# dingliumath/MCMC.jl

Hardware: AMD Instinct MI355X
Metric: MCMC steps*chains/sec (1M chains, d=32) (higher is better)
Workload: dtype f64; 1 GPU; metric: d=32 iso-Normal, RWM(0.1), 2^20 chains/GPU (BASELINE metric); SerialMC(steps=2967, burnin=296, thinning=10), 1048576 chains/GPU, RWM; d=32, chains_per_gpu=1048576, global_chains=1048576, sampler=rwm, burnin=296, thinning=10, kept_per_chain=268, steps_per_launch=0, evals=3111124992, key=metric|d=32|chains=1048576|rwm|steps=2967|thinning=10|spl=0, parallelism=chains sharded over 1 GPU(s), no collective in the step loop

## Files before the change

### mcmc.jl_amd/csrc/detmath.hpp

```cpp
#pragma once
#include <hip/hip_runtime.h>
#include <stdint.h>

#include "bm_log_table.inc"
#include "erfc_table.inc"
#include "softplus_table.inc"

namespace mcmc {

enum : uint32_t { TAG_NORMAL = 0u, TAG_ACCEPT = 1u, TAG_NUTS_DOUBLING = 3u, TAG_NUTS_MERGE = 4u, TAG_DATA = 7u };

struct u32x4 { uint32_t x, y, z, w; };

template <bool U = false>
__device__ __forceinline__ u32x4 philox4x32_10(uint32_t c0, uint32_t c1, uint32_t c2, uint32_t c3,
                                               uint32_t k0, uint32_t k1) {
#pragma unroll
    for (int r = 0; r < 10; ++r) {
        if (r > 0) { k0 += 0x9E3779B9u; k1 += 0xBB67AE85u; }
        const uint64_t p0 = (uint64_t)0xD2511F53u * (uint64_t)c0;
        const uint64_t p1 = (uint64_t)0xCD9E8D57u * (uint64_t)c2;
        uint32_t n0, n2;
        if (U && r == 0) {
            n0 = (uint32_t)(p1 >> 32) ^ (c1 ^ k0);
// ... 99 lines not shown
    const double ln2_hi = 0x1.62e42fee00000p-1;
    const double ln2_lo = 0x1.a39ef35793c76p-33;
    const double shifter = 0x1.8p52;
    const double xc = __builtin_fmin(__builtin_fmax(x, -746.0), 710.0);
    const double t = __builtin_fma(xc, inv_ln2, shifter);
    const double kd = t - shifter;
    E.k = (int)kd;
    double r = __builtin_fma(-kd, ln2_hi, xc);
    E.r = __builtin_fma(-kd, ln2_lo, r);
    E.x = x;
    E.p = 0x1.6124613a86d09p-33;
}
__device__ __forceinline__ void det_exp_s2(ExpState& E) {
    double p = E.p;
    const double r = E.r;
    p = __builtin_fma(p, r, 0x1.1eed8eff8d898p-29);
    p = __builtin_fma(p, r, 0x1.ae64567f544e4p-26);
    p = __builtin_fma(p, r, 0x1.27e4fb7789f5cp-22);
    p = __builtin_fma(p, r, 0x1.71de3a556c734p-19);
    p = __builtin_fma(p, r, 0x1.a01a01a01a01ap-16);
    p = __builtin_fma(p, r, 0x1.a01a01a01a01ap-13);
    p = __builtin_fma(p, r, 0x1.6c16c16c16c17p-10);
    E.p = p;
}
__device__ __forceinline__ void det_exp_s3(ExpState& E) {
    double p = E.p;
    const double r = E.r;
    p = __builtin_fma(p, r, 0x1.1111111111111p-7);
    p = __builtin_fma(p, r, 0x1.5555555555555p-5);
    p = __builtin_fma(p, r, 0x1.5555555555555p-3);
    p = __builtin_fma(p, r, 0.5);
    p = __builtin_fma(p, r, 1.0);
    p = __builtin_fma(p, r, 1.0);
    E.p = p;
}
__device__ __forceinline__ double det_exp_fin(const ExpState& E) {
    const int k1 = E.k / 2, k2 = E.k - k1;
    double res = (E.p * pow2i(k1)) * pow2i(k2);
    const double x = E.x;
    if (x > 709.782712893384) res = __builtin_inf();
    if (x < -745.1332191019412) res = 0.0;
    if (x != x) res = x;
    return res;
}
__device__ __forceinline__ double det_exp(double x) {
    ExpState E;
    det_exp_s1(x, E);
    det_exp_s2(E);
    det_exp_s3(E);
    return det_exp_fin(E);
}

__device__ __forceinline__ void det_sincos2pi(double u, double& s_out, double& c_out) {
    const double q = __builtin_floor(__builtin_fma(u, 4.0, 0.5));
    const double r = __builtin_fma(q, -0.25, u);
    const double r2 = r * r;
    double S = -0x1.6fadb9f155744p-1;
    S = __builtin_fma(S, r2, 0x1.e8f434d018d63p+1);
    S = __builtin_fma(S, r2, -0x1.e3074fde8871fp+3);
    S = __builtin_fma(S, r2, 0x1.50783487ee782p+5);
    S = __builtin_fma(S, r2, -0x1.32d2cce62bd86p+6);
    S = __builtin_fma(S, r2, 0x1.466bc6775aae2p+6);
    S = __builtin_fma(S, r2, -0x1.4abbce625be53p+5);
    S = __builtin_fma(S, r2, 0x1.921fb54442d18p+2);
    double C = 0x1.20c62c2f2d7f5p-2;
    C = __builtin_fma(C, r2, -0x1.b6e24f44b128fp+0);
    C = __builtin_fma(C, r2, 0x1.f9d38a3763cc3p+2);
    C = __builtin_fma(C, r2, -0x1.a6d1f2a204a8cp+4);
    C = __builtin_fma(C, r2, 0x1.e1f506891babbp+5);
    C = __builtin_fma(C, r2, -0x1.55d3c7e3cbffap+6);
    C = __builtin_fma(C, r2, 0x1.03c1f081b5ac4p+6);
    C = __builtin_fma(C, r2, -0x1.3bd3cc9be45dep+4);
    C = __builtin_fma(C, r2, 1.0);
    const double sn = r * S;
    const int qi = ((int)q) & 3;
    const double a = (qi & 1) ? C : sn;
    const double b = (qi & 1) ? sn : C;
    s_out = (qi & 2) ? -a : a;
    c_out = (qi == 1 || qi == 2) ? -b : b;
}

static __device__ const double kBmLogTab[128][4] = {BM_LOG_TABLE_ROWS};
static __device__ const double kBmLog512Tab[512][4] = {BM_LOG512_TABLE_ROWS};

__device__ __forceinline__ double bm_log_u32(uint32_t w, const double (*tab)[4] = kBmLog512Tab) {
    const double ln2_hi = 0x1.62e42fee00000p-1;
    const double ln2_lo = 0x1.a39ef35793c76p-33;
    const double x = (double)w + 0.5;
    const uint64_t b = d2bits(x);
    const uint32_t xh = (uint32_t)(b >> 32);
    const uint32_t up = (xh >> 19) & 1u;
    const int e = (int)(xh >> 20) + (int)up - (1023 + 32);
    const uint32_t mhi = ((0x3ffu ^ up) << 20) | (xh & 0x000fffffu);
    const double m = bits2d(((uint64_t)mhi << 32) | (b & 0xffffffffull));
    typedef double f64x2_t __attribute__((ext_vector_type(2)));
    const f64x2_t* row = reinterpret_cast<const f64x2_t*>(reinterpret_cast<const char*>(tab) + ((xh >> 6) & 0x3fe0u));
    const f64x2_t a = row[0], t = row[1];
    const double r = __builtin_fma(m, a.x, -1.0);
    double P = __builtin_fma(r, -0x1.5555555555555p-3, 0x1.999999999999ap-3);
    P = __builtin_fma(r, P, -0x1p-2);
    P = __builtin_fma(r, P, 0x1.5555555555555p-2);
    P = __builtin_fma(r, P, -0x1p-1);
    const double p = __builtin_fma(r * r, P, r);
    const double de = (double)e;
    const double hi = __builtin_fma(de, ln2_hi, a.y);
    const double lo = __builtin_fma(de, ln2_lo, t.x) + p;
    return hi + lo;
}

static __device__ const double kBmRad512Tab[512][4] = {BM_RAD512_TABLE_ROWS};

__device__ __forceinline__ double bm_rad2_u32(uint32_t w, const double (*tab)[4] = kBmRad512Tab) {
    const double m2ln2_hi = -0x1.62e42fee00000p+0;
    const double m2ln2_lo = -0x1.a39ef35793c76p-32;
    const double x = (double)w + 0.5;
    const uint64_t b = d2bits(x);
    const uint32_t xh = (uint32_t)(b >> 32);
    const uint32_t up = (xh >> 19) & 1u;
    const int e = (int)(xh >> 20) + (int)up - (1023 + 32);
    const uint32_t mhi = ((0x3ffu ^ up) << 20) | (xh & 0x000fffffu);
    const double m = bits2d(((uint64_t)mhi << 32) | (b & 0xffffffffull));
    typedef double f64x2_t __attribute__((ext_vector_type(2)));
    const f64x2_t* row = reinterpret_cast<const f64x2_t*>(reinterpret_cast<const char*>(tab) + ((xh >> 6) & 0x3fe0u));
    const f64x2_t a = row[0], t = row[1];
    const double r2 = __builtin_fma(m, a.x, 2.0);
    double Q = __builtin_fma(r2, 0x1.5555555555555p-8, 0x1.999999999999ap-7);
    Q = __builtin_fma(r2, Q, 0x1p-5);
    Q = __builtin_fma(r2, Q, 0x1.5555555555555p-4);
    Q = __builtin_fma(r2, Q, 0x1p-2);
    const double p2 = __builtin_fma(r2 * r2, Q, r2);
    const double de = (double)e;
    const double hi = __builtin_fma(de, m2ln2_hi, a.y);
    const double lo = __builtin_fma(de, m2ln2_lo, t.x) + p2;
    return hi + lo;
}

static __device__ const double kBmRadPTab[4 * BM_RADP_NROWS][2] = {BM_RADP_TABLE_ROWS};
static __device__ const double kBmRadTTab[4 * BM_RADT_NROWS][2] = {BM_RADT_TABLE_ROWS};

struct RadTab {
    const double (*d)[2];
    bool lds;
};
__device__ __forceinline__ RadTab rad_tab_global() { return RadTab{kBmRadPTab, false}; }

__device__ __forceinline__ double bm_radius_u32(uint32_t w, RadTab rt) {
    typedef double f64x2_t __attribute__((ext_vector_type(2)));
    const uint32_t sm = (uint32_t)((int32_t)w >> 31);
    const uint32_t v = w ^ sm;
    const double y = (double)v;
    const uint64_t b = d2bits(y);
    const uint32_t yh = (uint32_t)(b >> 32);
    const bool tail = v < (1u << 21);
    constexpr uint32_t kOff0 = 0u - ((uint32_t)((1023 + 21) << 5) << 4);
    constexpr uint32_t kOff1 = kOff0 + (uint32_t)(BM_RADP_NROWS / 2) * 16u;
    uint32_t sel;
    asm("v_bfi_b32 %0, %1, %2, %3" : "=v"(sel) : "v"(sm), "v"(kOff1), "s"(kOff0));
    uint32_t off;
    asm("v_lshl_add_u32 %0, %1, 4, %2" : "=v"(off) : "v"(yh >> 15), "v"(sel));
    uint32_t th = yh;
    asm("v_and_or_b32 %0, %0, %1, %2" : "+v"(th) : "s"(0x7fffu), "v"(0x3ff00000u));
    if (!rt.lds) off = tail ? 0u : off;
    double t = bits2d(((uint64_t)th << 32) | (b & 0xffffffffull)) - (1.0 + 1.0 / 64.0);
    const char* base = reinterpret_cast<const char*>(rt.d) + off;
    f64x2_t c0 = *reinterpret_cast<const f64x2_t*>(base);
    f64x2_t c1 = *reinterpret_cast<const f64x2_t*>(base + 16 * BM_RADP_NROWS);
    f64x2_t c2 = *reinterpret_cast<const f64x2_t*>(base + 32 * BM_RADP_NROWS);
    f64x2_t c3 = *reinterpret_cast<const f64x2_t*>(base + 48 * BM_RADP_NROWS);
    if (tail) {
        uint32_t vv = v;
        asm volatile("" : "+v"(vv));
        const double x = (double)vv + 0.5;
        const uint64_t bx = d2bits(x);
        const uint32_t xh = (uint32_t)(bx >> 32);
        const uint32_t rw = (uint32_t)((int)(xh >> 15) - ((1023 - 1) << 5)) * 16u + (sm & (16u * (BM_RADT_NROWS / 2)));
        t = bits2d(((uint64_t)((xh & 0x7fffu) | 0x3ff00000u) << 32) | (bx & 0xffffffffull)) - (1.0 + 1.0 / 64.0);
        asm volatile(
            "global_load_dwordx4 %0, %4, %5\n\t"
            "global_load_dwordx4 %1, %4, %6\n\t"
            "global_load_dwordx4 %2, %4, %7\n\t"
            "global_load_dwordx4 %3, %4, %8\n\t"
            "s_waitcnt vmcnt(0)"
            : "=&v"(c0), "=&v"(c1), "=&v"(c2), "=&v"(c3)
            : "v"(rw), "s"(&kBmRadTTab[0][0]), "s"(&kBmRadTTab[BM_RADT_NROWS][0]),
              "s"(&kBmRadTTab[2 * BM_RADT_NROWS][0]), "s"(&kBmRadTTab[3 * BM_RADT_NROWS][0])
            : "memory");
    }
    double q = __builtin_fma(c3.y, t, c3.x);
    q = __builtin_fma(q, t, c2.y);
    q = __builtin_fma(q, t, c2.x);
    q = __builtin_fma(q, t, c1.y);
    q = __builtin_fma(q, t, c1.x);
    q = __builtin_fma(q, t, c0.y);
    double r = __builtin_fma(q, t, c0.x);
    asm volatile("" : "+v"(r));
    return r;
}

typedef double dm_f64x2 __attribute__((ext_vector_type(2)));

static __device__ const double kExp2Tab[64][2] = {EXP2_TABLE_ROWS};

struct ExpTState {
    double x, r, em;
    dm_f64x2 t;
    int e;
};
__device__ __forceinline__ void det_exp_tab_s1(double x, ExpTState& E, const double (*tab)[2] = kExp2Tab) {
    const double k64 = 0x1.71547652b82fep+6;
    const double l_hi = 0x1.62e42fee00000p-7;
    const double l_lo = 0x1.a39ef35793c76p-39;
    const double shifter = 0x1.8p52;
    const double xc = __builtin_fmin(__builtin_fmax(x, -746.0), 710.0);
    const double kd = __builtin_fma(xc, k64, shifter) - shifter;
    const int k = (int)kd;
    E.t = *reinterpret_cast<const dm_f64x2*>(tab[k & 63]);
    E.e = k >> 6;
    const double r = __builtin_fma(-kd, l_hi, xc);
    E.r = __builtin_fma(-kd, l_lo, r);
    E.x = x;
}
__device__ __forceinline__ void det_exp_tab_s2(ExpTState& E) {
    const double r = E.r;
    double P = __builtin_fma(r, 0x1.6c16c16c16c17p-10, 0x1.1111111111111p-7);
    P = __builtin_fma(r, P, 0x1.5555555555555p-5);
    P = __builtin_fma(r, P, 0x1.5555555555555p-3);
    P = __builtin_fma(r, P, 0.5);
    P = __builtin_fma(r, P, 1.0);
    E.em = r * P;
}
__device__ __forceinline__ double det_exp_tab_fin(const ExpTState& E) {
    const int e1 = E.e / 2, e2 = E.e - e1;
    double res = E.t.x + __builtin_fma(E.t.x, E.em, E.t.y);
    res = (res * pow2i(e1)) * pow2i(e2);
    return E.x != E.x ? E.x : res;
}
__device__ __forceinline__ double det_exp_tab(double x, const double (*tab)[2] = kExp2Tab) {
    ExpTState E;
    det_exp_tab_s1(x, E, tab);
    det_exp_tab_s2(E);
    return det_exp_tab_fin(E);
}

struct LogTState {
    double v, m, p;
    dm_f64x2 a, t;
    int e;
};
#ifndef GLM_LOG_FREXP
#define GLM_LOG_FREXP 0
#endif
__device__ __forceinline__ void det_log_tab_s1(double v, LogTState& L, const double (*tab)[4] = kBmLogTab) {
#if GLM_LOG_FREXP
    const double mh = __builtin_amdgcn_frexp_mant(v);
    const int eh = __builtin_amdgcn_frexp_exp(v);
    const uint64_t b = d2bits(mh);
    const uint32_t top7 = (uint32_t)(b >> 45) & 0x7fu;
    const uint32_t up = top7 >> 6;
    L.e = eh - 1 + (int)up;
    L.m = bits2d((b & 0x000fffffffffffffull) | ((uint64_t)(0x3ffu - up) << 52));
    const dm_f64x2* row = reinterpret_cast<const dm_f64x2*>(tab[top7]);
    L.a = row[0];
    L.t = row[1];
    L.v = v;
#else
    const bool sub = v < 0x1p-1022;
    const double xs = sub ? v * 0x1p54 : v;
    const uint64_t b = d2bits(xs);
    const uint32_t top7 = (uint32_t)(b >> 45) & 0x7fu;
    const uint32_t up = top7 >> 6;
    L.e = (int)(uint32_t)(b >> 52) - 1023 + (int)up - (sub ? 54 : 0);
    L.m = bits2d((b & 0x000fffffffffffffull) | ((uint64_t)(0x3ffu - up) << 52));
    const dm_f64x2* row = reinterpret_cast<const dm_f64x2*>(tab[top7]);
    L.a = row[0];
    L.t = row[1];
    L.v = v;
#endif
}
__device__ __forceinline__ void det_log_tab_s2(LogTState& L) {
    const double r = __builtin_fma(L.m, L.a.x, -1.0);
    double P = __builtin_fma(r, -0x1p-3, 0x1.2492492492492p-3);
    P = __builtin_fma(r, P, -0x1.5555555555555p-3);
    P = __builtin_fma(r, P, 0x1.999999999999ap-3);
    P = __builtin_fma(r, P, -0x1p-2);
    P = __builtin_fma(r, P, 0x1.5555555555555p-2);
    P = __builtin_fma(r, P, -0x1p-1);
    L.p = __builtin_fma(r * r, P, r);
}
__device__ __forceinline__ double det_log_tab_fin(const LogTState& L) {
    const double ln2_hi = 0x1.62e42fee00000p-1;
    const double ln2_lo = 0x1.a39ef35793c76p-33;
    const double de = (double)L.e;
    const double hi = __builtin_fma(de, ln2_hi, L.a.y);
    const double lo = __builtin_fma(de, ln2_lo, L.t.x) + L.p;
    const double res = L.v == 0.0 ? -__builtin_inf() : hi + lo;
    return L.v != L.v ? L.v : res;
}
__device__ __forceinline__ double det_log_tab(double v, const double (*tab)[4] = kBmLogTab) {
    LogTState L;
    det_log_tab_s1(v, L, tab);
    det_log_tab_s2(L);
    return det_log_tab_fin(L);
}

static __device__ const double kSoftplusTab[SP_NROWS][10] = {SP_TABLE_ROWS};


struct LogiState {
    double u, t, p, d;
    const dm_f64x2* row;
};
__device__ __forceinline__ void det_logi_s1(double eta, double w, LogiState& S, const double (*tab)[10] = kSoftplusTab) {
    const double shifter = 0x1.8p52;
    const double u = -(w * eta);
    const double vs = __builtin_fmin(__builtin_fabs(u), (double)SP_VMAX);
    const double tt = __builtin_fma(vs, (double)SP_SEG, shifter);
    const uint32_t j = (uint32_t)d2bits(tt);
    const double kd = tt - shifter;
    S.t = __builtin_fma(-kd, 1.0 / SP_SEG, vs);
    S.row = reinterpret_cast<const dm_f64x2*>(tab[j]);
    S.u = u;
}
__device__ __forceinline__ void det_logi_s2(LogiState& S) {
    const double t = S.t;
    const dm_f64x2 c89 = S.row[4], c67 = S.row[3], c45 = S.row[2];
    double p = c89.y, d = c89.y;
    p = __builtin_fma(p, t, c89.x);
    d = __builtin_fma(d, t, p); p = __builtin_fma(p, t, c67.y);
    d = __builtin_fma(d, t, p); p = __builtin_fma(p, t, c67.x);
    d = __builtin_fma(d, t, p); p = __builtin_fma(p, t, c45.y);
    d = __builtin_fma(d, t, p); p = __builtin_fma(p, t, c45.x);
    S.p = p;
    S.d = d;
}
__device__ __forceinline__ void det_logi_fin(const LogiState& S, double w, double& term, double& rv) {
    const double t = S.t;
    const dm_f64x2 c23 = S.row[1], c01 = S.row[0];
    double p = S.p, d = S.d;
    d = __builtin_fma(d, t, p); p = __builtin_fma(p, t, c23.y);
    d = __builtin_fma(d, t, p); p = __builtin_fma(p, t, c23.x);
    d = __builtin_fma(d, t, p); p = __builtin_fma(p, t, c01.y);
    d = __builtin_fma(d, t, p); p = __builtin_fma(p, t, c01.x);
    term = -(__builtin_fmax(S.u, 0.0) + p);
    const double sig = S.u >= 0.0 ? 1.0 + d : -d;
    rv = w * sig;
}
__device__ __forceinline__ void det_logi(double eta, double w, double& term, double& rv,
                                         const double (*tab)[10] = kSoftplusTab) {
    LogiState S;
    det_logi_s1(eta, w, S, tab);
    det_logi_s2(S);
    det_logi_fin(S, w, term, rv);
}

static __device__ const double kBmSinCos1024Tab[1024][2] = {BM_SINCOS1024_TABLE_ROWS};

constexpr double kSinJ1 = 0x1.921fb54442d18p-30, kSinJ3 = -0x1.4abbce625be53p-91, kSinJ5 = 0x1.466bc6775aae2p-154;
constexpr double kCosJ2 = -0x1.3bd3cc9be45dep-60, kCosJ4 = 0x1.03c1f081b5ac4p-122;

__device__ __forceinline__ void det_sincos2pi_u32(uint32_t w, double& s_out, double& c_out,
                                                  const double (*sct)[2] = kBmSinCos1024Tab) {
    const int32_t ji = ((int32_t)(w << 10)) >> 10;
    const uint32_t off = (w - (uint32_t)ji) >> 18;
    const double j = (double)ji;
    const double j2 = j * j;
    const double sr = j * __builtin_fma(j2, __builtin_fma(j2, kSinJ5, kSinJ3), kSinJ1);
    const double cr = __builtin_fma(j2, __builtin_fma(j2, kCosJ4, kCosJ2), 1.0);
    typedef double f64x2_t __attribute__((ext_vector_type(2)));
    const f64x2_t a = *reinterpret_cast<const f64x2_t*>(reinterpret_cast<const char*>(sct) + off);
    s_out = __builtin_fma(a.x, cr, a.y * sr);
    c_out = __builtin_fma(a.y, cr, -(a.x * sr));
}

__device__ __forceinline__ double sqrt_pos_normal(double x) {
    const double y = __builtin_amdgcn_rsq(x);
    double g = x * y;
    double h = 0.5 * y;
    const double r = __builtin_fma(-h, g, 0.5);
    g = __builtin_fma(g, r, g);
    h = __builtin_fma(h, r, h);
    double e = __builtin_fma(-g, g, x);
    g = __builtin_fma(e, h, g);
    e = __builtin_fma(-g, g, x);
    return __builtin_fma(e, h, g);
}

__device__ __forceinline__ void normals4(const u32x4& w, double& z0, double& z1, double& z2, double& z3,
                                         RadTab rt = rad_tab_global(),
                                         const double (*sct)[2] = kBmSinCos1024Tab) {
    {
        const double rad = bm_radius_u32(w.x, rt);
        double s, c;
        det_sincos2pi_u32(w.y, s, c, sct);
        z0 = rad * c; z1 = rad * s;
    }
    {
        const double rad = bm_radius_u32(w.z, rt);
        double s, c;
        det_sincos2pi_u32(w.w, s, c, sct);
        z2 = rad * c; z3 = rad * s;
    }
    asm volatile("" : "+v"(z0), "+v"(z1), "+v"(z2), "+v"(z3));
}

__device__ __attribute__((noinline)) bool gt_det_log_exact(double ratio, double u) { return ratio > det_log(u); }
__device__ __forceinline__ bool gt_det_log(double ratio, double u) {
    const double L = (double)__builtin_amdgcn_logf((float)u) * 0x1.62e42fefa39efp-1;
    const double E = 0x1p-16 * (1.0 + __builtin_fabs(L));
    const bool sure_acc = ratio > L + E;
    const bool sure_rej = ratio <= L - E;
    bool acc = sure_acc;
    if (!sure_acc && !sure_rej) acc = gt_det_log_exact(ratio, u);
    return acc;
}

__device__ __forceinline__ double round_away(double x) {
    double t = __builtin_trunc(x);
    const double fr = x - t;
    if (fr >= 0.5) t += 1.0;
    else if (fr <= -0.5) t -= 1.0;
    return t;
}

static __device__ const double kErfcTaylor[14] = {ERFC_TAYLOR_COEFS};
static __device__ const double kErfcPoly[32][13] = {ERFC_POLY_ROWS};
__device__ __forceinline__ double det_erfcx_ge_half(double x) {
    if (x >= 128.0) {
        const double v = 1.0 / (x * x);
        const double s = __builtin_fma(__builtin_fma(__builtin_fma(v, -1.875, 0.75), v, -0.5), v, 1.0);
        return s / (x * 0x1.c5bf891b4ef6bp+0);
    }
    const uint64_t bx = d2bits(x);
    const uint32_t hx = (uint32_t)(bx >> 32);
    const int i = (int)(hx >> 18) - (1022 << 2);
    const double c = bits2d((uint64_t)((hx & 0xfffc0000u) | 0x00020000u) << 32);
    const double sc = bits2d((uint64_t)(2046u - (hx >> 20) + 3u) << 52);
    const double t = (x - c) * sc;
    const double* P = kErfcPoly[i];
    double p = P[12];
#pragma unroll
    for (int n = 11; n >= 0; --n) p = __builtin_fma(p, t, P[n]);
    return p;
}
__device__ __forceinline__ double det_erfc(double a) {
    const double x = __builtin_fabs(a);
    double r;
    if (x < 0.5) {
        const double u = x * x;
        double q = kErfcTaylor[13];
#pragma unroll
        for (int n = 12; n >= 0; --n) q = __builtin_fma(q, u, kErfcTaylor[n]);
        r = 1.0 - x * q;
    } else if (x < 32.0) {
        const double p = det_erfcx_ge_half(x);
        const double xh = bits2d(d2bits(x) & 0xfffffffff8000000ull);
        const double e1 = det_exp(-(xh * xh));
        const double e2 = det_exp(-((x - xh) * (x + xh)));
        r = (e1 * e2) * p;
    } else {
        r = 0.0;
    }
    r = a < 0.0 ? 2.0 - r : r;
    return a != a ? a : r;
}
__device__ __forceinline__ double det_log1p(double t) {
    const double u = 1.0 + t;
    return u == 1.0 ? t : det_log(u) * (t / (u - 1.0));
}
__device__ __forceinline__ double det_normlogcdf(double z) {
    const double invsqrt2 = 0x1.6a09e667f3bcdp-1;
    const double r = z < -1.0 ? det_log(det_erfcx_ge_half(-z * invsqrt2) / 2.0) - (z * z) / 2.0
                              : det_log1p(-det_erfc(z * invsqrt2) / 2.0);
    return z != z ? z : r;
}

}
```

### mcmc.jl_amd/csrc/samplers.hpp

```cpp
#pragma once
#include "common.hpp"
#include "detmath.hpp"
#include "models.hpp"
#include "ram.hpp"
#include "host/kernels_api.hpp"

namespace mcmc {

constexpr int kBlock = 256;

enum TabMode : int { kTabLds = 0, kTabGlobal = 1 };

struct BmLds {
    double (*rd)[2];
    double (*sc)[2];
};
__device__ __forceinline__ BmLds bm_lds_tables() {
    __shared__ __attribute__((aligned(16))) double lds_radd[4 * BM_RADP_NROWS][2];
    __shared__ __attribute__((aligned(16))) double lds_sct[1024][2];
    return BmLds{lds_radd, lds_sct};
}

template <int NT>
__device__ __forceinline__ void stage_bm_tables(const BmLds& L) {
    typedef double f64x2_t __attribute__((ext_vector_type(2)));
    constexpr int kD = 4 * BM_RADP_NROWS, kS = 1024;
    constexpr int kU = kD + kS;
    constexpr int kN = (kU + NT - 1) / NT;
    constexpr int kBatch = 8;
    const f64x2_t* gd = reinterpret_cast<const f64x2_t*>(&kBmRadPTab[0][0]);
    const f64x2_t* gs = reinterpret_cast<const f64x2_t*>(&kBmSinCos1024Tab[0][0]);
    f64x2_t* ld = reinterpret_cast<f64x2_t*>(&L.rd[0][0]);
    f64x2_t* ls = reinterpret_cast<f64x2_t*>(&L.sc[0][0]);
#pragma unroll
    for (int j0 = 0; j0 < kN; j0 += kBatch) {
        f64x2_t v[kBatch];
#pragma unroll
        for (int j = j0; j < j0 + kBatch && j < kN; ++j) {
            const int u = (int)threadIdx.x + NT * j;
            if (u < kU) v[j - j0] = u < kD ? gd[u] : gs[u - kD];
        }
#pragma unroll
        for (int j = j0; j < j0 + kBatch && j < kN; ++j) {
            const int u = (int)threadIdx.x + NT * j;
            if (u < kD) ld[u] = v[j - j0];
            else if (u < kU) ls[u - kD] = v[j - j0];
        }
    }
    __syncthreads();
}

template <int TAB, int NT>
struct BmTables {
    RadTab rad;
    const double (*sct)[2];
    BmLds lds;
    __device__ __forceinline__ void init() {
        if constexpr (TAB == kTabLds) {
            lds = bm_lds_tables();
            rad = RadTab{lds.rd, true};
            sct = lds.sc;
        } else {
            rad = rad_tab_global();
            sct = kBmSinCos1024Tab;
        }
    }
    __device__ __forceinline__ void stage() const {
        if constexpr (TAB == kTabLds) stage_bm_tables<NT>(lds);
    }
};

template <int NB_, bool FULL = false, bool SPLIT = false, int TH = kBlock, int TAB = kTabGlobal>
struct LaneChain {
    static constexpr int NB = NB_;
    static constexpr int NC = 4 * NB_;
    static constexpr int kSplit = SPLIT ? 4 * ((NB_ + 1) / 2) : 0;
    static constexpr int kThreads = TH;
    static constexpr int kChainsPerBlock = TH;
    static constexpr bool kPairs = false;
    int64_t c;
    bool live;
    int d;
    BmTables<TAB, TH> bt;
    __device__ LaneChain(const StepArgs& s, bool defer = false) {
        c = (int64_t)blockIdx.x * TH + threadIdx.x;
        live = c < s.C;
        d = s.d;
        bt.init();
        if (!defer) stage();
    }
    __device__ __forceinline__ void stage() const { bt.stage(); }
    __device__ __forceinline__ int coord(int k) const { return k; }
    __device__ __forceinline__ bool valid(int k) const { return FULL || k < 4 * (NB - 1) || k < d; }
    __device__ __forceinline__ uint32_t block(int b) const { return (uint32_t)b; }
    __device__ __forceinline__ double reduce(double v) const { return v; }
    __device__ __forceinline__ bool any(bool v) const { return v; }
    __device__ __forceinline__ void load(const double* x, int64_t ld, double (&v)[NC]) const {
        uint64_t o = (uint64_t)(live ? c : 0);
#pragma unroll
        for (int k = 0; k < NC; ++k) {
            v[k] = valid(k) ? x[o] : 0.0;
            o += (uint64_t)ld;
            asm volatile("" : "+v"(o));
        }
    }
    __device__ __forceinline__ void store(double* x, int64_t ld, const double (&v)[NC]) const {
        if (!live) return;
        uint64_t o = (uint64_t)c;
#pragma unroll
        for (int k = 0; k < NC; ++k) {
            if (valid(k)) x[o] = v[k];
            o += (uint64_t)ld;
            asm volatile("" : "+v"(o));
        }
    }
    __device__ __forceinline__ double load_scalar(const double* p) const { return p[live ? c : 0]; }
    template <class T>
    __device__ __forceinline__ T load_t(const T* p) const { return p[live ? c : 0]; }
    template <class T>
    __device__ __forceinline__ void store_t(T* p, T v) const {
        if (live) p[c] = v;
    }
    __device__ __forceinline__ void store_kept(const StepArgs& s, int64_t kk, const double (&v)[NC],
                                               double* base) const {
        if (base == nullptr || !live) return;
        double* p = base + (size_t)kk * (size_t)d * (size_t)s.C;
        const uint64_t C = (uint64_t)s.C;
        uint64_t o = (uint64_t)c;
#pragma unroll
        for (int k = 0; k < NC; ++k) {
            if (valid(k)) p[o] = v[k];
            o += C;
            asm volatile("" : "+v"(o));
        }
    }
    __device__ __forceinline__ void store_cm(const StepArgs& s, int64_t l, const double (&v)[NC], double* base) const {
        store_kept(s, l, v, base);
    }
    __device__ __forceinline__ void count_evals(const StepArgs& s, int64_t n) const {
        if (s.n_evals == nullptr) return;
        unsigned long long v = live ? (unsigned long long)n : 0ull;
#pragma unroll
        for (int off = 32; off >= 1; off >>= 1) v += __shfl_xor(v, off, 64);
        if ((threadIdx.x & 63) == 0) atomicAdd(s.n_evals, v);
    }
    __device__ __forceinline__ void store_bit(const StepArgs& s, int64_t kk, bool acc) const {
        const uint64_t mask = __ballot(acc && live);
        if ((threadIdx.x & 63) == 0 && s.acc_bits != nullptr) {
            const int64_t w = c >> 6;
            if (w < s.nw) s.acc_bits[(size_t)kk * (size_t)s.nw + (size_t)w] = mask;
        }
    }
};

template <int NB_, bool FULL = false, int TH = 512, int TAB = kTabLds>
struct PairChain {
    static constexpr int NB = NB_;
    static constexpr int NC = 4 * NB_;
    static constexpr int kThreads = TH;
    static constexpr int kChainsPerBlock = TH / 2;
    static constexpr bool kPairs = true;
    int64_t c;
    bool live;
    int d;
    int h;
    BmTables<TAB, TH> bt;
    __device__ PairChain(const StepArgs& s, bool defer = false) {
        const int lane = (int)(threadIdx.x & 63);
        c = (int64_t)blockIdx.x * kChainsPerBlock + (int64_t)(threadIdx.x >> 6) * 32 + (lane & 31);
        h = lane >> 5;
        live = c < s.C;
        d = s.d;
        bt.init();
        if (!defer) stage();
    }
    __device__ __forceinline__ void stage() const { bt.stage(); }
    __device__ __forceinline__ static uint32_t tid_now() {
        uint32_t t = threadIdx.x;
        asm volatile("" : "+v"(t));
        return t;
    }
    __device__ __forceinline__ int64_t c_now() const {
        const uint32_t t = tid_now();
        return (int64_t)blockIdx.x * kChainsPerBlock + (int64_t)((t >> 6) * 32 + (t & 31));
    }
    __device__ __forceinline__ int coord(int k) const { return h * NC + k; }
    __device__ __forceinline__ bool valid(int k) const { return FULL || coord(k) < d; }
    __device__ __forceinline__ uint32_t block(int b) const { return (uint32_t)(h * NB + b); }
    __device__ __forceinline__ double from_half(double v, int which) const {
        const uint64_t u = (uint64_t)__double_as_longlong(v);
        const uint32_t lo = (uint32_t)u, hi = (uint32_t)(u >> 32);
        const auto a = __builtin_amdgcn_permlane32_swap(lo, lo, false, false);
        const auto b = __builtin_amdgcn_permlane32_swap(hi, hi, false, false);
        return which == 0 ? __longlong_as_double((long long)(((uint64_t)b[0] << 32) | a[0]))
                          : __longlong_as_double((long long)(((uint64_t)b[1] << 32) | a[1]));
    }
    __device__ __forceinline__ double reduce(double v) const {
        const uint64_t u = (uint64_t)__double_as_longlong(v);
        const uint32_t lo = (uint32_t)u, hi = (uint32_t)(u >> 32);
        const auto a = __builtin_amdgcn_permlane32_swap(lo, lo, false, false);
        const auto b = __builtin_amdgcn_permlane32_swap(hi, hi, false, false);
        const double v0 = __longlong_as_double((long long)(((uint64_t)b[0] << 32) | a[0]));
        const double v1 = __longlong_as_double((long long)(((uint64_t)b[1] << 32) | a[1]));
        return v0 + v1;
    }
    __device__ __forceinline__ bool any(bool v) const {
        const uint64_t m = __ballot(v);
        const int l = (int)(threadIdx.x & 31);
        return (((m >> l) | (m >> (l + 32))) & 1ull) != 0;
    }
    __device__ __forceinline__ void load(const double* x, int64_t ld, double (&v)[NC]) const {
        uint64_t o = (uint64_t)(live ? c : 0) + (uint64_t)(h * NC) * (uint64_t)ld;
#pragma unroll
        for (int k = 0; k < NC; ++k) {
            v[k] = valid(k) ? x[o] : 0.0;
            o += (uint64_t)ld;
            asm volatile("" : "+v"(o));
        }
    }
    __device__ __forceinline__ void store(double* x, int64_t ld, const double (&v)[NC]) const {
        if (!live) return;
        const int hn = (int)((tid_now() >> 5) & 1);
        uint64_t o = (uint64_t)c_now() + (uint64_t)(hn * NC) * (uint64_t)ld;
#pragma unroll
        for (int k = 0; k < NC; ++k) {
            if (valid(k)) x[o] = v[k];
            o += (uint64_t)ld;
            asm volatile("" : "+v"(o));
        }
    }
    __device__ __forceinline__ double load_scalar(const double* p) const { return p[live ? c : 0]; }
    template <class T>
    __device__ __forceinline__ T load_t(const T* p) const { return p[live ? c : 0]; }
    template <class T>
    __device__ __forceinline__ void store_t(T* p, T v) const {
        if (live && h == 0) p[c_now()] = v;
    }
    __device__ __forceinline__ void store_kept(const StepArgs& s, int64_t kk, const double (&v)[NC],
                                               double* base) const {
        if (base == nullptr || !live) return;
        const uint64_t C = (uint64_t)s.C;
        const uint32_t lo = (uint32_t)((uint64_t)c * 8u + (uint64_t)(h * NC) * C * 8u);
        char* row = reinterpret_cast<char*>(base + (size_t)kk * (size_t)d * (size_t)C);
#pragma unroll
        for (int k = 0; k < NC; ++k) {
            if (valid(k)) *reinterpret_cast<double*>(row + lo) = v[k];
            row += C * 8u;
        }
    }
    __device__ __forceinline__ void store_cm(const StepArgs& s, int64_t l, const double (&v)[NC], double* base) const {
        store_kept(s, l, v, base);
    }
    __device__ __forceinline__ void count_evals(const StepArgs& s, int64_t n) const {
        if (s.n_evals == nullptr) return;
        unsigned long long v = (live && h == 0) ? (unsigned long long)n : 0ull;
#pragma unroll
        for (int off = 32; off >= 1; off >>= 1) v += __shfl_xor(v, off, 64);
        if ((threadIdx.x & 63) == 0) atomicAdd(s.n_evals, v);
    }
    __device__ __forceinline__ void store_bit(const StepArgs& s, int64_t kk, bool acc) const {
        const uint64_t mask = __ballot(acc && live);
        if ((threadIdx.x & 63) == 0 && s.acc_bits != nullptr) {
            const int64_t cc = c_now();
            const int64_t w = cc >> 6;
            if (w < s.nw)
                reinterpret_cast<uint32_t*>(s.acc_bits)[((size_t)kk * (size_t)s.nw + (size_t)w) * 2 + (size_t)((cc >> 5) & 1)] =
                    (uint32_t)mask;
        }
    }
};

__device__ __forceinline__ double wave_sum(double v) {
#pragma unroll
    for (int off = 32; off >= 1; off >>= 1) v = v + __shfl_xor(v, off, 64);
    return v;
}

template <int W>
__device__ __forceinline__ double block_sum(double v) {
    v = wave_sum(v);
    if (W == 1) return v;
    __shared__ double part[W];
    if ((threadIdx.x & 63) == 0) part[threadIdx.x >> 6] = v;
    __syncthreads();
    double t = part[0];
#pragma unroll
    for (int w = 1; w < W; ++w) t = t + part[w];
    __syncthreads();
    return t;
}

template <int G, bool FULL = false, int W = 1, int TAB = kTabGlobal>
struct WaveChain {
    static constexpr int NB = G;
    static constexpr int NC = 4 * G;
    static constexpr bool kPairs = false;
    static constexpr int L = 64 * W;
    int64_t c;
    bool live;
    int d;
    int lane;
    int64_t ldr;
    BmTables<TAB, W == 1 ? kBlock : 64 * W> bt;
    __device__ WaveChain(const StepArgs& s, bool defer = false) {
        c = W == 1 ? (int64_t)blockIdx.x * (kBlock / 64) + (threadIdx.x >> 6) : (int64_t)blockIdx.x;
        live = c < s.C;
        d = s.d;
        lane = W == 1 ? (int)(threadIdx.x & 63) : (int)threadIdx.x;
        ldr = s.ld;
        bt.init();
        if (!defer) stage();
    }
    __device__ __forceinline__ void stage() const { bt.stage(); }
    __device__ __forceinline__ int coord(int k) const { return 4 * (lane + L * (k >> 2)) + (k & 3); }
    __device__ __forceinline__ bool valid(int k) const { return FULL || coord(k) < d; }
    __device__ __forceinline__ uint32_t block(int b) const { return (uint32_t)(lane + L * b); }
    __device__ __forceinline__ double reduce(double v) const { return block_sum<W>(v); }
    __device__ __forceinline__ bool any(bool v) const { return W == 1 ? __ballot(v) != 0 : __syncthreads_or(v) != 0; }
    __device__ __forceinline__ void load(const double* x, int64_t , double (&v)[NC]) const {
        const double* row = x + (size_t)(live ? c : 0) * (size_t)ldr;
#pragma unroll
        for (int g = 0; g < G; ++g) {
            const int j0 = 4 * (lane + L * g);
            if (FULL || j0 < d) {
                const double4 q = *reinterpret_cast<const double4*>(row + j0);
                v[4 * g] = q.x; v[4 * g + 1] = q.y; v[4 * g + 2] = q.z; v[4 * g + 3] = q.w;
            } else {
                v[4 * g] = v[4 * g + 1] = v[4 * g + 2] = v[4 * g + 3] = 0.0;
            }
        }
#pragma unroll
        for (int k = 0; k < NC; ++k)
            if (!valid(k)) v[k] = 0.0;
    }
    __device__ __forceinline__ void store(double* x, int64_t , const double (&v)[NC]) const {
        if (!live) return;
        double* row = x + (size_t)c * (size_t)ldr;
#pragma unroll
        for (int g = 0; g < G; ++g) {
            const int j0 = 4 * (lane + L * g);
            if (FULL || j0 < d) *reinterpret_cast<double4*>(row + j0) = make_double4(v[4 * g], v[4 * g + 1], v[4 * g + 2],
                                                                               v[4 * g + 3]);
        }
    }
    __device__ __forceinline__ double load_scalar(const double* p) const { return p[live ? c : 0]; }
    template <class T>
    __device__ __forceinline__ T load_t(const T* p) const { return p[live ? c : 0]; }
    template <class T>
    __device__ __forceinline__ void store_t(T* p, T v) const {
        if (live && lane == 0) p[c] = v;
    }
    __device__ __forceinline__ void store_kept(const StepArgs& s, int64_t kk, const double (&v)[NC],
                                               double* base) const {
        if (base == nullptr || !live) return;
        double* row = base + ((size_t)kk * (size_t)s.C + (size_t)c) * (size_t)ldr;
#pragma unroll
        for (int g = 0; g < G; ++g) {
            const int j0 = 4 * (lane + L * g);
            if (FULL || j0 < d) *reinterpret_cast<double4*>(row + j0) = make_double4(v[4 * g], v[4 * g + 1], v[4 * g + 2],
                                                                               v[4 * g + 3]);
        }
    }
    __device__ __forceinline__ void count_evals(const StepArgs& s, int64_t n) const {
        if (s.n_evals != nullptr && live && lane == 0) atomicAdd(s.n_evals, (unsigned long long)n);
    }
    __device__ __forceinline__ void store_cm(const StepArgs& s, int64_t l, const double (&v)[NC], double* base) const {
        if (base == nullptr || !live) return;
        double* p = base + (size_t)l * (size_t)d * (size_t)s.C + (size_t)c;
#pragma unroll
        for (int k = 0; k < NC; ++k)
            if (valid(k)) p[(size_t)coord(k) * (size_t)s.C] = v[k];
    }
    __device__ __forceinline__ void store_bit(const StepArgs& s, int64_t kk, bool acc) const {
        if (live && lane == 0 && acc && s.acc_bits != nullptr)
            atomicOr((unsigned long long*)&s.acc_bits[(size_t)kk * (size_t)s.nw + (size_t)(c >> 6)],
                     1ull << (c & 63));
    }
};

template <class P>
__device__ __forceinline__ void gen_normals(const P& p, const Stream& rs, uint32_t chain, uint32_t step,
                                            double (&z)[P::NC]) {
#pragma unroll
    for (int b = 0; b < P::NB; ++b) {
        const u32x4 w = rs.block_us(chain, step, p.block(b), TAG_NORMAL);
        normals4(w, z[4 * b], z[4 * b + 1], z[4 * b + 2], z[4 * b + 3], p.bt.rad, p.bt.sct);
    }
}


template <class P>
struct split_of { static constexpr int value = 0; };
template <int NB, bool F, bool S, int T, int TAB>
struct split_of<LaneChain<NB, F, S, T, TAB>> { static constexpr int value = LaneChain<NB, F, S, T, TAB>::kSplit; };

template <class P, class M>
__device__ __forceinline__ double eval_lp(const P& p, const M& model, const double (&v)[P::NC], bool& oos) {
    if constexpr (is_joint<M>::value) return model.joint_lp(v, oos);
    constexpr int S = split_of<P>::value;
    if constexpr (S > 0) {
        double a = 0.0, b = 0.0;
#pragma unroll
        for (int k = 0; k < P::NC; ++k)
            if (p.valid(k)) {
                if (k < S) model.acc(a, v[k]);
                else model.acc(b, v[k]);
            }
        return llacc_finish(model, a + b, oos);
    }
    double a = 0.0;
#pragma unroll
    for (int k = 0; k < P::NC; ++k)
        if (p.valid(k)) model.acc(a, v[k]);
    return llacc_finish(model, p.reduce(a), oos);
}

template <class M, int NC, bool J = is_joint<M>::value>
struct GradAt {
    const M& m;
    __device__ __forceinline__ GradAt(const M& model, const double (&)[NC], bool = true) : m(model) {}
    __device__ __forceinline__ double operator()(int, double v) const { return m.grad(v); }
};
template <class M, int NC>
struct GradAt<M, NC, true> {
    double g[NC];
    __device__ __forceinline__ GradAt(const M& model, const double (&v)[NC], bool need = true) {
        if (need) {
            model.joint_grad(v, g);
        } else {
#pragma unroll
            for (int k = 0; k < NC; ++k) g[k] = 0.0;
        }
    }
    __device__ __forceinline__ double operator()(int k, double) const { return g[k]; }
};

template <class P>
__device__ __forceinline__ double half_dot(const P& p, const double (&m)[P::NC]) {
    double a = 0.0;
#pragma unroll
    for (int k = 0; k < P::NC; ++k)
        if (p.valid(k)) a = __builtin_fma(m[k], m[k], a);
    return 0.5 * p.reduce(a);
}

__device__ __forceinline__ bool mh_accept_short_circuit(const Stream& rs, uint32_t chain, uint32_t step, double ratio) {
    bool acc = ratio > 0.0;
    if (!acc) {
        const u32x4 w = rs.block(chain, step, 0u, TAG_ACCEPT);
        acc = gt_det_log(ratio, uniform52(w.x, w.y));
    }
    return acc;
}

template <class P>
struct AcceptDraw {
    double u_next = 0.0;
    __device__ __forceinline__ bool test(const P& p, const Stream& rs, uint32_t chain, int64_t i, int t, double ratio) {
        if constexpr (P::kPairs) {
            double u;
            if ((t & 1) == 0) {
                const u32x4 w = rs.block(chain, (uint32_t)(i + p.h), 0u, TAG_ACCEPT);
                const double uu = uniform52(w.x, w.y);
                u = p.from_half(uu, 0);
                u_next = uu;
            } else {
                u = p.from_half(u_next, 1);
            }
            bool acc = ratio > 0.0;
            if (!acc) acc = gt_det_log(ratio, u);
            return acc;
        } else {
            return mh_accept_short_circuit(rs, chain, (uint32_t)i, ratio);
        }
    }
};

__device__ __forceinline__ double tune_factor(int32_t acc, int32_t prop, double target) {
    const double rate = (double)acc / (double)prop;
    return 1.0 / (1.0 + det_exp(-11.0 * (rate - target))) + 0.5;
}

struct Keeper {
    int64_t next;
    int64_t kk;
    int64_t thin;
    int32_t left;
    __device__ explicit Keeper(const StepArgs& s) {
        thin = s.thinning;
        const int64_t lo = s.step_begin - s.run_step0;
        const int64_t hi = lo + s.nsteps - 1;
        int64_t first = s.burnin + 1;
        if (lo > first) first += ((lo - first + thin - 1) / thin) * thin;
        const int64_t last = hi < s.len ? hi : s.len;
        if (first > last) {
            next = -1; kk = 0; left = 0;
        } else {
            next = s.run_step0 + first;
            kk = (first - s.burnin - 1) / thin;
            left = (int32_t)((last - first) / thin);
        }
    }
    __device__ __forceinline__ bool take(int64_t i, int64_t* out) {
        if (i != next) return false;
        *out = kk;
        if (left > 0) { next += thin; kk += 1; left -= 1; } else next = -1;
        return true;
    }
};

template <class P, class M, bool US = false>
__device__ __forceinline__ void rwm_body(const KernelArgs& a) {
    const StepArgs& s = a.s;
    const P p(s, true);
    const M model(a.m);
    const Stream rs{s.key0, s.key1};
    const uint32_t chain = s.chain0 + (uint32_t)p.c;
    double x[P::NC], sc[P::NC];
    p.load(a.st.x, s.ld, x);
    double lp = p.load_scalar(a.st.lp);
    p.stage();
#pragma unroll
    for (int k = 0; k < P::NC; ++k) sc[k] = p.valid(k) ? (US ? s.scale1 : s.scale[p.coord(k)]) : 0.0;
    AcceptDraw<P> ad;

    Keeper keep(s);
    for (int t = 0; t < s.nsteps; ++t) {
        const int64_t i = s.step_begin + t;
        double xp[P::NC];
        gen_normals(p, rs, chain, (uint32_t)i, xp);
#pragma unroll
        for (int k = 0; k < P::NC; ++k) xp[k] = x[k] + xp[k] * sc[k];
        bool oos;
        const double lpp = eval_lp(p, model, xp, oos);
        const double ratio = lpp - lp;
        const bool acc = ad.test(p, rs, chain, i, t, ratio);
        if (acc) {
#pragma unroll
            for (int k = 0; k < P::NC; ++k) x[k] = xp[k];
            lp = lpp;
        }
        int64_t kk;
        if (keep.take(i, &kk)) {
            p.store_kept(s, kk, x, s.samples);
            p.store_bit(s, kk, acc);
        }
    }
    p.store(a.st.x, s.ld, x);
    p.store_t(a.st.lp, lp);
    p.count_evals(s, s.nsteps);
}

template <class P, class M>
__device__ __forceinline__ void mala_body(const KernelArgs& a) {
    const StepArgs& s = a.s;
    const SamplerArgs& sa = a.sa;
    const P p(s);
    const M model(a.m);
    const Stream rs{s.key0, s.key1};
    const uint32_t chain = s.chain0 + (uint32_t)p.c;
    double x[P::NC];
    p.load(a.st.x, s.ld, x);
    double lp = p.load_scalar(a.st.lp);
    double h = sa.tuner ? p.load_scalar(a.st.t_step) : sa.drift_step;
    int32_t n_acc = sa.tuner ? p.load_t(a.st.t_acc) : 0;
    int32_t n_prop = sa.tuner ? p.load_t(a.st.t_prop) : 0;
    AcceptDraw<P> ad;

    Keeper keep(s);
    for (int t = 0; t < s.nsteps; ++t) {
        const int64_t i = s.step_begin + t;
        if (sa.tuner) n_prop += 1;
        const double half = h / 2.0;
        const double sq = __builtin_sqrt(h);
        const double twoh = 2.0 * h;
        const double L = det_log(kTwoPi * h) / 2.0;
        double xp[P::NC];
        gen_normals(p, rs, chain, (uint32_t)i, xp);
        double qf = 0.0;
        const GradAt<M, P::NC> gx(model, x);
#pragma unroll
        for (int k = 0; k < P::NC; ++k) {
            const double pm = x[k] + half * gx(k, x[k]);
            xp[k] = pm + sq * xp[k];
            const double e = pm - xp[k];
            if (p.valid(k)) qf = qf + ((-(e * e)) / twoh - L);
        }
        qf = p.reduce(qf);
        bool oos;
        const double lpp = eval_lp(p, model, xp, oos);
        double qb = 0.0;
        const GradAt<M, P::NC> gxp(model, xp, !oos);
#pragma unroll
        for (int k = 0; k < P::NC; ++k) {
            const double gp = oos ? 0.0 : gxp(k, xp[k]);
            const double e = (xp[k] + half * gp) - x[k];
            if (p.valid(k)) qb = qb + ((-(e * e)) / twoh - L);
        }
        qb = p.reduce(qb);
        const double ratio = ((lpp + qb) - lp) - qf;
        const bool acc = ad.test(p, rs, chain, i, t, ratio);
        if (acc) {
#pragma unroll
            for (int k = 0; k < P::NC; ++k) x[k] = xp[k];
            lp = lpp;
            if (sa.tuner) n_acc += 1;
        }
        int64_t kk;
        if (keep.take(i, &kk)) {
            p.store_kept(s, kk, x, s.samples);
            if (s.grads != nullptr) {
                double g[P::NC];
                const GradAt<M, P::NC> gk(model, x);
#pragma unroll
                for (int k = 0; k < P::NC; ++k) g[k] = gk(k, x[k]);
                p.store_kept(s, kk, g, s.grads);
            }
            p.store_bit(s, kk, acc);
        }
        if (sa.tuner && i <= s.tuner_burnin && (i % sa.adapt_step) == 0) {
            h = h * tune_factor(n_acc, n_prop, sa.target_rate);
            n_acc = 0;
            n_prop = 0;
        }
    }
    p.store(a.st.x, s.ld, x);
    p.store_t(a.st.lp, lp);
    p.count_evals(s, s.nsteps);
    if (sa.tuner) {
        p.store_t(a.st.t_step, h);
        p.store_t(a.st.t_acc, n_acc);
        p.store_t(a.st.t_prop, n_prop);
    }
}

template <class P, class M>
__device__ __forceinline__ double trajectory(const P& p, const M& model, double eps, int64_t nl, double (&x)[P::NC],
                                             double (&m)[P::NC]) {
    constexpr bool kCarry = P::NC <= 16;
    static_assert(kCarry || !is_joint<M>::value, "joint models run lane per chain (NC <= 16)");
    bool oos = false;
    double lpl = 0.0;
    double kick[kCarry ? P::NC : 1];
    if constexpr (kCarry) {
        const GradAt<M, P::NC> g0(model, x);
#pragma unroll
        for (int k = 0; k < P::NC; ++k) kick[k] = (0.5 * g0(k, x[k])) * eps;
    }
    for (int64_t l = 0; l < nl; ++l) {
#pragma unroll
        for (int k = 0; k < P::NC; ++k) {
            double a;
            if constexpr (kCarry) a = kick[k];
            else a = (0.5 * (oos ? 0.0 : model.grad(x[k]))) * eps;
            m[k] = m[k] + a;
            x[k] = x[k] + eps * m[k];
        }
        if (M::kLLAcc) lpl = eval_lp(p, model, x, oos);
        const GradAt<M, P::NC> gl(model, x, !oos);
#pragma unroll
        for (int k = 0; k < P::NC; ++k) {
            const double g = oos ? 0.0 : gl(k, x[k]);
            const double a = (0.5 * g) * eps;
            if constexpr (kCarry) kick[k] = a;
            m[k] = m[k] + a;
        }
    }
    if (!M::kLLAcc && nl > 0) lpl = eval_lp(p, model, x, oos);
    return lpl;
}

template <class P, class M>
__device__ __forceinline__ double trajectory_halfneg(const P& p, const M& model, double eps, int64_t nl,
                                                     double (&x)[P::NC], double (&m)[P::NC], bool& big) {
    double kick[P::NC];
    double xmax = 0.0;
#pragma unroll
    for (int k = 0; k < P::NC; ++k) {
        kick[k] = (-x[k]) * eps;
        xmax = __builtin_fmax(xmax, __builtin_fabs(x[k]));
    }
    for (int64_t l = 0; l < nl; ++l) {
#pragma unroll
// ... 317 lines not shown
```

Measured before the change: 32.49 billion chain-steps/s.

## Trim instructions in Box-Muller radius, sincos constants, accept test and lane swaps

Several micro-optimisations land together in the RWM inner loop. The radius lookup now uses a masked row index with a bias folded into the base pointer, plus a 2.0 inline constant and an fma-by-0.5, in place of a v_bfi select and a subtract. Two sincos polynomial constants are pinned in VGPRs across the step loop for paired-lane chains. The accept fast-path now tests with one subtract and one fma-based error bound. The permlane32 swap for the paired uniform is done once per two steps, producing both halves together instead of swapping on every step. LDS tables are merged into one struct and h is recomputed from tid, which may change register pressure.

```diff
diff --git a/mcmc.jl_amd/csrc/detmath.hpp b/mcmc.jl_amd/csrc/detmath.hpp
--- a/mcmc.jl_amd/csrc/detmath.hpp
+++ b/mcmc.jl_amd/csrc/detmath.hpp
@@ -275,17 +275,15 @@
     const uint64_t b = d2bits(y);
     const uint32_t yh = (uint32_t)(b >> 32);
     const bool tail = v < (1u << 21);
-    constexpr uint32_t kOff0 = 0u - ((uint32_t)((1023 + 21) << 5) << 4);
-    constexpr uint32_t kOff1 = kOff0 + (uint32_t)(BM_RADP_NROWS / 2) * 16u;
-    uint32_t sel;
-    asm("v_bfi_b32 %0, %1, %2, %3" : "=v"(sel) : "v"(sm), "v"(kOff1), "s"(kOff0));
+    constexpr uint32_t kRowBias = (uint32_t)(((1023 + 21) << 5) & 0x1ff) * 16u;
+    const uint32_t sel = sm & ((uint32_t)(BM_RADP_NROWS / 2) * 16u);
     uint32_t off;
-    asm("v_lshl_add_u32 %0, %1, 4, %2" : "=v"(off) : "v"(yh >> 15), "v"(sel));
+    asm("v_lshl_add_u32 %0, %1, 4, %2" : "=v"(off) : "v"((yh >> 15) & 0x1ffu), "v"(sel));
     uint32_t th = yh;
-    asm("v_and_or_b32 %0, %0, %1, %2" : "+v"(th) : "s"(0x7fffu), "v"(0x3ff00000u));
-    if (!rt.lds) off = tail ? 0u : off;
-    double t = bits2d(((uint64_t)th << 32) | (b & 0xffffffffull)) - (1.0 + 1.0 / 64.0);
-    const char* base = reinterpret_cast<const char*>(rt.d) + off;
+    asm("v_and_or_b32 %0, %0, %1, 2.0" : "+v"(th) : "s"(0x7fffu));
+    if (!rt.lds) off = tail ? kRowBias : off;
+    double m2 = bits2d(((uint64_t)th << 32) | (b & 0xffffffffull));
+    const char* base = reinterpret_cast<const char*>(rt.d) + off - kRowBias;
     f64x2_t c0 = *reinterpret_cast<const f64x2_t*>(base);
     f64x2_t c1 = *reinterpret_cast<const f64x2_t*>(base + 16 * BM_RADP_NROWS);
     f64x2_t c2 = *reinterpret_cast<const f64x2_t*>(base + 32 * BM_RADP_NROWS);
@@ -297,7 +295,7 @@
         const uint64_t bx = d2bits(x);
         const uint32_t xh = (uint32_t)(bx >> 32);
         const uint32_t rw = (uint32_t)((int)(xh >> 15) - ((1023 - 1) << 5)) * 16u + (sm & (16u * (BM_RADT_NROWS / 2)));
-        t = bits2d(((uint64_t)((xh & 0x7fffu) | 0x3ff00000u) << 32) | (bx & 0xffffffffull)) - (1.0 + 1.0 / 64.0);
+        m2 = bits2d(((uint64_t)((xh & 0x7fffu) | 0x40000000u) << 32) | (bx & 0xffffffffull));
         asm volatile(
             "global_load_dwordx4 %0, %4, %5\n\t"
             "global_load_dwordx4 %1, %4, %6\n\t"
@@ -309,6 +307,8 @@
               "s"(&kBmRadTTab[2 * BM_RADT_NROWS][0]), "s"(&kBmRadTTab[3 * BM_RADT_NROWS][0])
             : "memory");
     }
+    double t;
+    asm("v_fma_f64 %0, %1, 0.5, %2" : "=v"(t) : "v"(m2), "s"(-(1.0 + 1.0 / 64.0)));
     double q = __builtin_fma(c3.y, t, c3.x);
     q = __builtin_fma(q, t, c2.y);
     q = __builtin_fma(q, t, c2.x);
@@ -481,14 +481,24 @@
 constexpr double kSinJ1 = 0x1.921fb54442d18p-30, kSinJ3 = -0x1.4abbce625be53p-91, kSinJ5 = 0x1.466bc6775aae2p-154;
 constexpr double kCosJ2 = -0x1.3bd3cc9be45dep-60, kCosJ4 = 0x1.03c1f081b5ac4p-122;
 
+struct AngleK {
+    double s3 = kSinJ3, c2 = kCosJ2;
+    __device__ __forceinline__ static AngleK resident() {
+        AngleK k;
+        asm volatile("" : "+v"(k.s3), "+v"(k.c2));
+        return k;
+    }
+};
+
 __device__ __forceinline__ void det_sincos2pi_u32(uint32_t w, double& s_out, double& c_out,
-                                                  const double (*sct)[2] = kBmSinCos1024Tab) {
+                                                  const double (*sct)[2] = kBmSinCos1024Tab,
+                                                  const AngleK& ak = AngleK{}) {
     const int32_t ji = ((int32_t)(w << 10)) >> 10;
     const uint32_t off = (w - (uint32_t)ji) >> 18;
     const double j = (double)ji;
     const double j2 = j * j;
-    const double sr = j * __builtin_fma(j2, __builtin_fma(j2, kSinJ5, kSinJ3), kSinJ1);
-    const double cr = __builtin_fma(j2, __builtin_fma(j2, kCosJ4, kCosJ2), 1.0);
+    const double sr = j * __builtin_fma(j2, __builtin_fma(j2, kSinJ5, ak.s3), kSinJ1);
+    const double cr = __builtin_fma(j2, __builtin_fma(j2, kCosJ4, ak.c2), 1.0);
     typedef double f64x2_t __attribute__((ext_vector_type(2)));
     const f64x2_t a = *reinterpret_cast<const f64x2_t*>(reinterpret_cast<const char*>(sct) + off);
     s_out = __builtin_fma(a.x, cr, a.y * sr);
@@ -510,17 +520,17 @@
 
 __device__ __forceinline__ void normals4(const u32x4& w, double& z0, double& z1, double& z2, double& z3,
                                          RadTab rt = rad_tab_global(),
-                                         const double (*sct)[2] = kBmSinCos1024Tab) {
+                                         const double (*sct)[2] = kBmSinCos1024Tab, const AngleK& ak = AngleK{}) {
     {
         const double rad = bm_radius_u32(w.x, rt);
         double s, c;
-        det_sincos2pi_u32(w.y, s, c, sct);
+        det_sincos2pi_u32(w.y, s, c, sct, ak);
         z0 = rad * c; z1 = rad * s;
     }
     {
         const double rad = bm_radius_u32(w.z, rt);
         double s, c;
-        det_sincos2pi_u32(w.w, s, c, sct);
+        det_sincos2pi_u32(w.w, s, c, sct, ak);
         z2 = rad * c; z3 = rad * s;
     }
     asm volatile("" : "+v"(z0), "+v"(z1), "+v"(z2), "+v"(z3));
@@ -529,11 +539,10 @@
 __device__ __attribute__((noinline)) bool gt_det_log_exact(double ratio, double u) { return ratio > det_log(u); }
 __device__ __forceinline__ bool gt_det_log(double ratio, double u) {
     const double L = (double)__builtin_amdgcn_logf((float)u) * 0x1.62e42fefa39efp-1;
-    const double E = 0x1p-16 * (1.0 + __builtin_fabs(L));
-    const bool sure_acc = ratio > L + E;
-    const bool sure_rej = ratio <= L - E;
-    bool acc = sure_acc;
-    if (!sure_acc && !sure_rej) acc = gt_det_log_exact(ratio, u);
+    const double d = ratio - L;
+    const double E = __builtin_fma(__builtin_fabs(L), 0x1p-16, 0x1p-16);
+    bool acc = d > 0.0;
+    if (!(__builtin_fabs(d) > E)) acc = gt_det_log_exact(ratio, u);
     return acc;
 }
 
diff --git a/mcmc.jl_amd/csrc/samplers.hpp b/mcmc.jl_amd/csrc/samplers.hpp
--- a/mcmc.jl_amd/csrc/samplers.hpp
+++ b/mcmc.jl_amd/csrc/samplers.hpp
@@ -16,9 +16,12 @@
     double (*sc)[2];
 };
 __device__ __forceinline__ BmLds bm_lds_tables() {
-    __shared__ __attribute__((aligned(16))) double lds_radd[4 * BM_RADP_NROWS][2];
-    __shared__ __attribute__((aligned(16))) double lds_sct[1024][2];
-    return BmLds{lds_radd, lds_sct};
+    struct Tables {
+        double sct[1024][2];
+        double radd[4 * BM_RADP_NROWS][2];
+    };
+    __shared__ __attribute__((aligned(16))) Tables lds_bm;
+    return BmLds{lds_bm.radd, lds_bm.sct};
 }
 
 template <int NT>
@@ -184,24 +187,22 @@
         const uint32_t t = tid_now();
         return (int64_t)blockIdx.x * kChainsPerBlock + (int64_t)((t >> 6) * 32 + (t & 31));
     }
+    __device__ __forceinline__ static int h_now() { return (int)((tid_now() >> 5) & 1); }
     __device__ __forceinline__ int coord(int k) const { return h * NC + k; }
     __device__ __forceinline__ bool valid(int k) const { return FULL || coord(k) < d; }
     __device__ __forceinline__ uint32_t block(int b) const { return (uint32_t)(h * NB + b); }
-    __device__ __forceinline__ double from_half(double v, int which) const {
-        const uint64_t u = (uint64_t)__double_as_longlong(v);
-        const uint32_t lo = (uint32_t)u, hi = (uint32_t)(u >> 32);
-        const auto a = __builtin_amdgcn_permlane32_swap(lo, lo, false, false);
-        const auto b = __builtin_amdgcn_permlane32_swap(hi, hi, false, false);
-        return which == 0 ? __longlong_as_double((long long)(((uint64_t)b[0] << 32) | a[0]))
-                          : __longlong_as_double((long long)(((uint64_t)b[1] << 32) | a[1]));
+    __device__ __forceinline__ void halves(double v, double& v0, double& v1) const {
+        double w = v;
+        asm("" : "+v"(w));
+        const uint64_t u = (uint64_t)__double_as_longlong(v), uw = (uint64_t)__double_as_longlong(w);
+        const auto a = __builtin_amdgcn_permlane32_swap((uint32_t)u, (uint32_t)uw, false, false);
+        const auto b = __builtin_amdgcn_permlane32_swap((uint32_t)(u >> 32), (uint32_t)(uw >> 32), false, false);
+        v0 = __longlong_as_double((long long)(((uint64_t)b[0] << 32) | a[0]));
+        v1 = __longlong_as_double((long long)(((uint64_t)b[1] << 32) | a[1]));
     }
     __device__ __forceinline__ double reduce(double v) const {
-        const uint64_t u = (uint64_t)__double_as_longlong(v);
-        const uint32_t lo = (uint32_t)u, hi = (uint32_t)(u >> 32);
-        const auto a = __builtin_amdgcn_permlane32_swap(lo, lo, false, false);
-        const auto b = __builtin_amdgcn_permlane32_swap(hi, hi, false, false);
-        const double v0 = __longlong_as_double((long long)(((uint64_t)b[0] << 32) | a[0]));
-        const double v1 = __longlong_as_double((long long)(((uint64_t)b[1] << 32) | a[1]));
+        double v0, v1;
+        halves(v, v0, v1);
         return v0 + v1;
     }
     __device__ __forceinline__ bool any(bool v) const {
@@ -220,8 +221,7 @@
     }
     __device__ __forceinline__ void store(double* x, int64_t ld, const double (&v)[NC]) const {
         if (!live) return;
-        const int hn = (int)((tid_now() >> 5) & 1);
-        uint64_t o = (uint64_t)c_now() + (uint64_t)(hn * NC) * (uint64_t)ld;
+        uint64_t o = (uint64_t)c_now() + (uint64_t)(h_now() * NC) * (uint64_t)ld;
 #pragma unroll
         for (int k = 0; k < NC; ++k) {
             if (valid(k)) x[o] = v[k];
@@ -234,7 +234,7 @@
     __device__ __forceinline__ T load_t(const T* p) const { return p[live ? c : 0]; }
     template <class T>
     __device__ __forceinline__ void store_t(T* p, T v) const {
-        if (live && h == 0) p[c_now()] = v;
+        if (live && h_now() == 0) p[c_now()] = v;
     }
     __device__ __forceinline__ void store_kept(const StepArgs& s, int64_t kk, const double (&v)[NC],
                                                double* base) const {
@@ -253,7 +253,7 @@
     }
     __device__ __forceinline__ void count_evals(const StepArgs& s, int64_t n) const {
         if (s.n_evals == nullptr) return;
-        unsigned long long v = (live && h == 0) ? (unsigned long long)n : 0ull;
+        unsigned long long v = (live && h_now() == 0) ? (unsigned long long)n : 0ull;
 #pragma unroll
         for (int off = 32; off >= 1; off >>= 1) v += __shfl_xor(v, off, 64);
         if ((threadIdx.x & 63) == 0) atomicAdd(s.n_evals, v);
@@ -380,11 +380,11 @@
 
 template <class P>
 __device__ __forceinline__ void gen_normals(const P& p, const Stream& rs, uint32_t chain, uint32_t step,
-                                            double (&z)[P::NC]) {
+                                            double (&z)[P::NC], const AngleK& ak = AngleK{}) {
 #pragma unroll
     for (int b = 0; b < P::NB; ++b) {
         const u32x4 w = rs.block_us(chain, step, p.block(b), TAG_NORMAL);
-        normals4(w, z[4 * b], z[4 * b + 1], z[4 * b + 2], z[4 * b + 3], p.bt.rad, p.bt.sct);
+        normals4(w, z[4 * b], z[4 * b + 1], z[4 * b + 2], z[4 * b + 3], p.bt.rad, p.bt.sct, ak);
     }
 }
 
@@ -461,11 +461,9 @@
             double u;
             if ((t & 1) == 0) {
                 const u32x4 w = rs.block(chain, (uint32_t)(i + p.h), 0u, TAG_ACCEPT);
-                const double uu = uniform52(w.x, w.y);
-                u = p.from_half(uu, 0);
-                u_next = uu;
+                p.halves(uniform52(w.x, w.y), u, u_next);
             } else {
-                u = p.from_half(u_next, 1);
+                u = u_next;
             }
             bool acc = ratio > 0.0;
             if (!acc) acc = gt_det_log(ratio, u);
@@ -523,12 +521,13 @@
 #pragma unroll
     for (int k = 0; k < P::NC; ++k) sc[k] = p.valid(k) ? (US ? s.scale1 : s.scale[p.coord(k)]) : 0.0;
     AcceptDraw<P> ad;
+    const AngleK ak = P::kPairs ? AngleK::resident() : AngleK{};
 
     Keeper keep(s);
     for (int t = 0; t < s.nsteps; ++t) {
         const int64_t i = s.step_begin + t;
         double xp[P::NC];
-        gen_normals(p, rs, chain, (uint32_t)i, xp);
+        gen_normals(p, rs, chain, (uint32_t)i, xp, ak);
 #pragma unroll
         for (int k = 0; k < P::NC; ++k) xp[k] = x[k] + xp[k] * sc[k];
         bool oos;
```

Result: faster. 33.01 billion chain-steps/s (median of 6 runs) (+1.6%).
